# aexoden/snesimage

Measured on AMD Instinct MI355X. Metric: candidate palettes scored/sec, higher is better.
Workload: dtype f32

## Files before the change

### snesimage_amd/csrc/capi.hip

```cpp
#include "../../include/snesimage_hip.h"
#include "kernels.hpp"
#include "kernels_opt.hpp"
#include "kernels_fast.hpp"
#include "kernels_sparse.hpp"
#include "kernels_sparse2.hpp"
#include "kernels_batch.hpp"
#include "kernels_shared.hpp"
#include "kernels_tile.hpp"
#include "kernels_level.hpp"
#include "kernels_char.hpp"
#include "kernels_char_set.hpp"
#include "kernels_guide.hpp"
#include "kernels_guide_lab.hpp"
#include "kernels_guide_window.hpp"
#include "kernels_guide_set_window.hpp"

#include <hip/hip_runtime.h>

#include <atomic>
#include <cmath>
#include <cstdio>
#include <cstdlib>
#include <cstring>
#include <string>
// ... 121 lines not shown
    std::vector<Lane> extra; uint32_t nlanes = 2; hipEvent_t ev_ready = nullptr;
    struct Sparse {
        bool lpt = true;
        bool down1 = true;
        bool counters_cleared = false;
        uint32_t h2q_max = 512;
        bool down_tiles = true;
        uint32_t h0_min = 1024;
        bool base_down_side = false;
        uint32_t h0_grid = 8192;
        hipStream_t h0_stream[8] = {}; hipEvent_t ev_scan[8] = {}, ev_h0[8] = {}, ev_hn[8] = {}, ev_vn[8] = {};
        bool v0_aside = true;
        hipEvent_t ev_v0[8] = {};
        bool vn_aside = true;
        uint32_t tiles_grid = 4096;
        uint32_t down1_grid = 32768;
        bool vsplit = true;
        uint32_t scan4_max = 2048;
        uint32_t hgrid = 8192;
        bool weight_mask = true;
        bool h_planes = true;
        bool debug_poison = false;
        bool dedup = true; uint32_t dedup_min = 1024; int *holder = nullptr; bool holder_dirty = false;
        bool enabled = false, side = true; uint32_t min_n = 1; uint32_t cap = 0, lanes = 0;
        SparseGeom S{};
        float *store = nullptr, *cand_tab = nullptr, *cand_lab = nullptr, *ckf = nullptr, *ckh = nullptr; long long zeros_off = 0; uint32_t *bitmap = nullptr; double *cka = nullptr, *part = nullptr;
        CandMeta *meta = nullptr; unsigned int *items = nullptr; int *item_count = nullptr; long long item_stride = 0; int *order = nullptr, *first = nullptr;
        uint4 *plist = nullptr; int *plist_count = nullptr; bool plist_valid = false;
        hipStream_t base_stream = nullptr; hipEvent_t ev_base_in = nullptr, ev_base_h = nullptr, ev_base_done = nullptr, ev_base_narrow = nullptr;
        uint8_t *dmaps = nullptr, *dmapsC4 = nullptr;
        uint8_t *bmap = nullptr, *bmapC4 = nullptr, *bcand = nullptr; unsigned long long *dpack = nullptr; double *ckd = nullptr; uint32_t slot_ci = 0;
        float *rec_lab = nullptr;
        int base_sp = -1, base_si = -1;
        struct Ahead { uint8_t *bmap = nullptr, *bmapC4 = nullptr, *bcand = nullptr; unsigned long long *dpack = nullptr; double *ckd = nullptr; float *btab = nullptr, *blab = nullptr, *rec_lab = nullptr; int *ok = nullptr;
                       hipEvent_t ev = nullptr; bool on = true, have = false; int sp = -1, si = -1; unsigned long long epoch = 0; } ahead;
    } sp;
    uint8_t *d_cand = nullptr; uint32_t cand_cap = 0;
    uint8_t *d_cand_sel = nullptr;
    double *d_errs = nullptr, *d_errs_sel = nullptr;
    double *d_inc_err = nullptr;
    StepResult *d_last = nullptr;
    double *d_scratch_err = nullptr;
    uint8_t *d_dummy_cand = nullptr;
    KmeansWork km{};
    double *d_tile_cost = nullptr; int *d_tile_any = nullptr; unsigned int *d_tile_moved = nullptr;

// ... 448 lines not shown
            Dn.orig = c->d_orig; Dn.tile_pal = c->d_tile_pal; Dn.pal_rgb8 = c->d_pal_rgb8; Dn.cand_tab = ah.btab; Dn.maps = ah.bmap; Dn.mapsC4 = ah.bmapC4;
            Dn.W = (int)c->W; Dn.H = (int)c->H; Dn.sub_size = (int)c->sub_size; Dn.ncol = c->ncol; Dn.slot_ci = (uint32_t)(np * (int)c->sub_size + ni);
            Dn.rec_pack = ah.dpack; Dn.ck_out = ah.ckd; Dn.excl_sub = np; Dn.excl_si = ni; Dn.excl_j0 = nj0;
            if (c->perceptual) {
                hipLaunchKernelGGL(k_candidate_lab, dim3(1), dim3(64), 0, bs, ah.btab, 1, c->d_lab_eotf, ah.blab);
                Dn.pal_lab = c->d_pal_lab; Dn.cand_lab = ah.blab; Dn.lab_eotf = c->d_lab_eotf; Dn.perceptual = 1; Dn.rec_lab = ah.rec_lab;
                if (c->dither4) hipLaunchKernelGGL((k_dither4_lab<1>), dim3(1), dim3(512), 0, bs, Dn); else hipLaunchKernelGGL((k_dither<true, 0, 1>), dim3(1), dim3(128), 0, bs, Dn);
            } else
            if (c->dither4 && c->sub_size == 15) hipLaunchKernelGGL((k_dither4<15, 1>), dim3(1), dim3(512), 0, bs, Dn);
            else if (c->dither4 && c->sub_size == 16) hipLaunchKernelGGL((k_dither4<16, 1>), dim3(1), dim3(512), 0, bs, Dn);
            else if (c->dither4) hipLaunchKernelGGL((k_dither4<0, 1>), dim3(1), dim3(512), 0, bs, Dn);
            else if (c->sub_size == 15) hipLaunchKernelGGL((k_dither<false, 15, 1>), dim3(1), dim3(128), 0, bs, Dn);
            else if (c->sub_size == 16) hipLaunchKernelGGL((k_dither<false, 16, 1>), dim3(1), dim3(128), 0, bs, Dn);
            else hipLaunchKernelGGL((k_dither<false, 0, 1>), dim3(1), dim3(128), 0, bs, Dn);
            HIPCHK(hipGetLastError());
            HIPCHK(hipEventRecord(ah.ev, bs));
            ah.have = true; ah.sp = np; ah.si = ni; ah.epoch = c->epoch;
        }
        sp.plist_valid = true;
    }
    return SNES_OK;
}

int32_t sparse_score_chunk(snesimage_ctx *c, uint32_t lane, hipStream_t stream, const uint8_t *d_rgb5, uint32_t nc, double *d_errors, int err_stride, int err_offset, int list0 = -1) {
    auto &sp = c->sp;
    const Geom &G = c->G;
    SparseParams P = sparse_params(c, lane);
    P.is_base = 0; P.ncand = (int)nc; P.k0 = (int)(lane * sp.cap);
    if (list0 >= 0) { P.holder = sp.holder; P.list0 = list0; }
    if (sp.debug_poison) HIPCHK(hipMemsetAsync(sp.store + (size_t)P.k0 * sp.S.cand_stride, 0xff, sizeof(float) * (size_t)sp.S.cand_stride * nc, stream));
    snesimage_ctx::TimingRec tr{}; tr.n = nc;
    if (c->timing) { for (int i = 0; i < 6; i++) HIPCHK(hipEventCreate(&tr.ev[i])); if (c->timing == 1) HIPCHK(hipEventRecord(tr.ev[0], stream)); }
    if (list0 >= 0) hipLaunchKernelGGL(k_candidate_tables_mark, dim3((nc + 63) / 64), dim3(64), 0, stream, d_rgb5, (int)nc, c->d_eotf, sp.cand_tab + 8 * (size_t)P.k0, sp.holder, list0);
    else
    hipLaunchKernelGGL(k_candidate_tables, dim3((nc + 63) / 64), dim3(64), 0, stream, d_rgb5, (int)nc, c->d_eotf, sp.cand_tab + 8 * (size_t)P.k0);
    if (c->dither) {
        if (c->perceptual) {
            hipLaunchKernelGGL(k_candidate_lab, dim3((nc + 63) / 64), dim3(64), 0, stream, sp.cand_tab + 8 * (size_t)P.k0, (int)nc, c->d_lab_eotf, sp.cand_lab + 3 * (size_t)P.k0);
            hipLaunchKernelGGL(k_dither_first_lab, dim3(nc), dim3(256), 0, stream, P);
        } else
        hipLaunchKernelGGL(k_dither_first, dim3((nc + 15) / 16), dim3(1024), 0, stream, P);
        DitherParams Dp{};
        Dp.orig = c->d_orig; Dp.tile_pal = c->d_tile_pal; Dp.pal_rgb8 = c->d_pal_rgb8; Dp.cand_tab = sp.cand_tab + 8 * (size_t)P.k0;
        Dp.maps = const_cast<uint8_t *>(P.maps); Dp.mapsC4 = const_cast<uint8_t *>(P.mapsC4);
        Dp.W = (int)c->W; Dp.H = (int)c->H; Dp.sub_size = (int)c->sub_size; Dp.ncol = c->ncol; Dp.slot_ci = sp.slot_ci;
        Dp.first_group = sp.first; Dp.first_k0 = P.k0; Dp.ck_in = sp.ckd; Dp.bmap = sp.bmap; Dp.bmapC4 = sp.bmapC4; Dp.rec_in = c->dither_rec ? sp.dpack : nullptr;
        if (c->sp.lpt) {
            hipLaunchKernelGGL(k_sparse_order, dim3(1), dim3(1024), 0, stream, P, sp.order + P.k0); Dp.order = sp.order + P.k0;
        }
        if (c->perceptual) {
            Dp.pal_lab = c->d_pal_lab; Dp.cand_lab = sp.cand_lab + 3 * (size_t)P.k0; Dp.lab_eotf = c->d_lab_eotf; Dp.perceptual = 1;
            if (c->dither4 && nc <= c->dither4_max) hipLaunchKernelGGL((k_dither4_lab<2>), dim3(nc), dim3(512), 0, stream, Dp); else hipLaunchKernelGGL((k_dither<true, 0, 2>), dim3(nc), dim3(128), 0, stream, Dp);
        } else
        if (c->dither4 && nc <= c->dither4_max && c->sub_size == 15) hipLaunchKernelGGL((k_dither4<15, 2>), dim3(nc), dim3(512), 0, stream, Dp);
        else if (c->dither4 && nc <= c->dither4_max && c->sub_size == 16) hipLaunchKernelGGL((k_dither4<16, 2>), dim3(nc), dim3(512), 0, stream, Dp);
        else if (c->dither4 && nc <= c->dither4_max) hipLaunchKernelGGL((k_dither4<0, 2>), dim3(nc), dim3(512), 0, stream, Dp);
// ... 71 lines not shown
    }
    if (vn_aside) {
        hipStream_t hs = sp.h0_stream[lane];
        HIPCHK(hipStreamWaitEvent(hs, sp.ev_hn[lane], 0));
        HIPCHK(hipStreamWaitEvent(hs, sp.ev_base_narrow, 0));
        hipLaunchKernelGGL(k_sparse_v, dim3((nc * 3 + 7) / 8, (unsigned)(G.nscales - P.s_first)), dim3(256), 0, hs, P);
        HIPCHK(hipEventRecord(sp.ev_vn[lane], hs));
    }
    if (v0_aside) {
        if (sp.side) HIPCHK(hipStreamWaitEvent(stream, sp.ev_base_narrow, 0));
        if (P.s_first < G.nscales) hipLaunchKernelGGL(k_sparse_v, dim3((nc * 3 + 7) / 8, (unsigned)(G.nscales - P.s_first)), dim3(256), 0, stream, P);
        if (P.s_first > 1) hipLaunchKernelGGL(k_sparse_v2_from, dim3(nc * 3, (unsigned)(P.s_first - 1)), dim3(256), 0, stream, P, 1);
    } else {
    if (c->timing) HIPCHK(hipEventRecord(tr.ev[3], stream));
    hipLaunchKernelGGL(k_sparse_v2, dim3(nc * 3, (unsigned)P.s_first), dim3(256), 0, stream, P);
    if (c->timing) HIPCHK(hipEventRecord(tr.ev[4], stream));
    }
    if (vn_aside) HIPCHK(hipStreamWaitEvent(stream, sp.ev_vn[lane], 0));
    else if (!v0_aside) {
    if (sp.side) HIPCHK(hipStreamWaitEvent(stream, sp.ev_base_narrow, 0));
    if (P.s_first < G.nscales) hipLaunchKernelGGL(k_sparse_v, dim3((nc * 3 + 7) / 8, (unsigned)(G.nscales - P.s_first)), dim3(256), 0, stream, P);
    }
    if (v0_aside) HIPCHK(hipStreamWaitEvent(stream, sp.ev_v0[lane], 0));
    hipLaunchKernelGGL(k_final_score_wave, dim3((nc + 3) / 4), dim3(256), 0, stream, sp.part + (size_t)P.k0 * G.nscales * 18, (int)nc, G, d_errors, err_stride, err_offset, P.item_count, (int)kItemLists);
    if (c->dither) {
        uint8_t *bm = lane == 0 ? c->d_bestmap : c->extra[lane - 1].d_bestmap; BestRec *br = lane == 0 ? c->d_bestrec : c->extra[lane - 1].d_bestrec;
        hipLaunchKernelGGL(k_keep_best, dim3(1), dim3(1024), 0, stream, d_errors, err_stride, err_offset, (int)nc, P.maps, (int)c->npx, br, bm);
    }
    HIPCHK(hipGetLastError());
    if (c->timing) { tr.light = c->timing != 1; if (!tr.light) HIPCHK(hipEventRecord(tr.ev[5], stream)); c->t_pending.push_back(tr); }
    return SNES_OK;
}

struct LaneScope {
    snesimage_ctx *c; snesimage_ctx::Lane *L;
    LaneScope(snesimage_ctx *c_, snesimage_ctx::Lane *L_) : c(c_), L(L_) { swap(); }
    ~LaneScope() { swap(); }
    void swap() { std::swap(c->stream, L->stream); std::swap(c->d_work, L->d_work); std::swap(c->d_cand_tab, L->d_cand_tab); std::swap(c->d_cand_lab, L->d_cand_lab);
                  std::swap(c->d_part, L->d_part); std::swap(c->d_maps, L->d_maps); std::swap(c->d_mapsT, L->d_mapsT); std::swap(c->d_mapsC4, L->d_mapsC4); std::swap(c->d_mapsR4, L->d_mapsR4);
                  std::swap(c->d_bestmap, L->d_bestmap); std::swap(c->d_bestrec, L->d_bestrec); }
};

int32_t score_list(snesimage_ctx *c, const uint8_t *d_rgb5, uint32_t n, double *d_errors, int err_stride, int err_offset, int sp, int si, uint8_t *d_maps_out) {
    uint32_t chunk = (c->dither || c->perceptual) ? (n + c->nlanes - 1) / c->nlanes : n;
    if (chunk < 64) chunk = 64;
    if (chunk > c->chunk) chunk = c->chunk;
    if (c->tied_call && chunk > 1024) chunk = 1024;
    const bool sparse = c->sp.enabled && !c->tied_call && !d_maps_out && sp >= 0 && n >= c->sp.min_n && c->pack_mode == (c->dither ? 1 : 2) && !(c->dither && c->sub_size == 1);
    const uint32_t nchunks = (n + chunk - 1) / chunk;
    const uint32_t nl = nchunks < c->nlanes ? nchunks : c->nlanes;
    CHECK(alloc_workspace(c, sparse ? 1 : chunk, nl));
    CHECK(ensure_tables(c));
    CHECK(ensure_source(c));
    if (sparse) {
        CHECK(sparse_alloc(c, chunk, nl));
        if (c->dither && (c->sp.base_sp != sp || c->sp.base_si != si)) c->sp.plist_valid = false;
        CHECK(sparse_base_pass(c, sp, si, n));
        c->sp.base_sp = sp; c->sp.base_si = si;
    }
    if (c->dither) { hipLaunchKernelGGL(k_reset_best, dim3(1), dim3(64), 0, c->stream, c->d_bestrecs_all, (int)c->nlanes); c->best_valid = true; }
    const bool dedup = sparse && !c->dither && c->sp.dedup && n >= c->sp.dedup_min;
    if (dedup) {
        if (!c->sp.holder) { HIPCHK(dmalloc(&c->sp.holder, sizeof(int) * kDedupColours)); c->sp.holder_dirty = true; }
        if (c->sp.holder_dirty) {
            HIPCHK(hipStreamSynchronize(c->stream));
            for (auto &L : c->extra) HIPCHK(hipStreamSynchronize(L.stream));
            HIPCHK(hipMemsetAsync(c->sp.holder, kNoHolder & 0xff, sizeof(int) * kDedupColours, c->stream));
        }
        c->sp.holder_dirty = true;
    }
    if (nl > 1) {
        HIPCHK(hipEventRecord(c->ev_ready, c->stream));
        for (uint32_t l = 1; l < nl; l++) HIPCHK(hipStreamWaitEvent(c->extra[l - 1].stream, c->ev_ready, 0));
    }
    uint32_t i = 0;
    for (uint32_t c0 = 0; c0 < n; c0 += chunk, i++) {
        const uint32_t nc = (n - c0 < chunk) ? (n - c0) : chunk;
        const uint32_t lane = i % nl;
        uint8_t *mo = d_maps_out ? d_maps_out + (size_t)c0 * c->npx : nullptr;
        const int eo = err_offset + (int)c0 * err_stride;
        if (sparse) { CHECK(sparse_score_chunk(c, lane, lane == 0 ? c->stream : c->extra[lane - 1].stream, d_rgb5 + 3 * (size_t)c0, nc, d_errors, err_stride, eo, dedup ? (int)c0 : -1)); continue; }
        if (lane == 0) CHECK(score_chunk(c, d_rgb5 + 3 * (size_t)c0, nc, d_errors, err_stride, eo, sp, si, mo));
        else { LaneScope ls(c, &c->extra[lane - 1]); CHECK(score_chunk(c, d_rgb5 + 3 * (size_t)c0, nc, d_errors, err_stride, eo, sp, si, mo)); }
    }
    for (uint32_t l = 1; l < nl; l++) {
        HIPCHK(hipEventRecord(c->extra[l - 1].done, c->extra[l - 1].stream));
        HIPCHK(hipStreamWaitEvent(c->stream, c->extra[l - 1].done, 0));
    }
    if (dedup) {
        hipLaunchKernelGGL(k_dedup_copy, dim3(1), dim3(1024), 0, c->stream, d_rgb5, (int)n, c->sp.holder, d_errors, err_stride, err_offset);
        HIPCHK(hipGetLastError());
        c->sp.holder_dirty = false;
    }
    return SNES_OK;
}

int32_t ensure_map(snesimage_ctx *c);

int32_t do_optimize(snesimage_ctx *c, bool may_skip = false) {
    CHECK(ensure_tables(c));
    if (!c->dither) {
        c->pack_valid = false;
        CHECK(run_prep(c, 0, -1, -1));
    } else {
        CHECK(alloc_workspace(c, 1));
        if (c->perceptual) CHECK(ensure_source(c));
        hipLaunchKernelGGL(k_candidate_tables, dim3(1), dim3(64), 0, c->stream, c->d_dummy_cand, 1, c->d_eotf, c->d_cand_tab);
        hipLaunchKernelGGL(k_candidate_slot, dim3(1), dim3(64), 0, c->stream, c->d_cand_tab, 1, 0xffffffffu);
        DitherParams Dp{};
        Dp.orig = c->d_orig; Dp.tile_pal = c->d_tile_pal; Dp.pal_rgb8 = c->d_pal_rgb8; Dp.pal_lab = c->d_pal_lab; Dp.cand_tab = c->d_cand_tab; Dp.cand_lab = c->d_cand_lab;
        Dp.lab_eotf = c->d_lab_eotf; Dp.maps = c->d_map; Dp.skip = may_skip ? c->d_skip : nullptr;
        Dp.W = (int)c->W; Dp.H = (int)c->H; Dp.sub_size = (int)c->sub_size; Dp.ncol = c->ncol; Dp.slot_ci = 0xffffffffu; Dp.perceptual = c->perceptual ? 1 : 0;
        launch_dither(c, Dp, 1);
// ... 165 lines not shown
    if (const char *e = getenv("SNES_BASE_STREAM")) c->sp.side = atoi(e) != 0;
    if (const char *e = getenv("SNES_LPT")) c->sp.lpt = atoi(e) != 0;
    if (const char *e = getenv("SNES_DOWN1")) c->sp.down1 = atoi(e) != 0;
    if (const char *e = getenv("SNES_DITHER4")) c->dither4 = atoi(e) != 0;
    if (const char *e = getenv("SNES_DITHERW")) c->ditherw = atoi(e) != 0;
    if (const char *e = getenv("SNES_DITHER_AHEAD")) c->sp.ahead.on = atoi(e) != 0;
    if (const char *e = getenv("SNES_DITHER_REC")) c->dither_rec = atoi(e) != 0;
    if (const char *e = getenv("SNES_DITHER4_MAX")) { int v = atoi(e); if (v >= 0) c->dither4_max = (uint32_t)v; }
    if (const char *e = getenv("SNES_DOWN1_GRID")) { int v = atoi(e); if (v >= 64) c->sp.down1_grid = (uint32_t)v; }
    if (const char *e = getenv("SNES_VSPLIT")) c->sp.vsplit = atoi(e) != 0;
    if (const char *e = getenv("SNES_DOWN_TILES")) c->sp.down_tiles = atoi(e) != 0;
    if (const char *e = getenv("SNES_V0_ASIDE")) c->sp.v0_aside = atoi(e) != 0;
    if (const char *e = getenv("SNES_VN_ASIDE")) c->sp.vn_aside = atoi(e) != 0;
    if (const char *e = getenv("SNES_H0_GRID")) { int v = atoi(e); if (v >= 16) c->sp.h0_grid = (uint32_t)v; }
    if (const char *e = getenv("SNES_H0_MIN")) { int v = atoi(e); if (v >= 0) c->sp.h0_min = (uint32_t)v; }
    if (const char *e = getenv("SNES_TILES_GRID")) { int v = atoi(e); if (v >= 64) c->sp.tiles_grid = (uint32_t)v; }
    if (const char *e = getenv("SNES_SCAN4_MAX")) { int v = atoi(e); if (v >= 0) c->sp.scan4_max = (uint32_t)v; }
    if (const char *e = getenv("SNES_H2Q_MAX")) { int v = atoi(e); if (v >= 0) c->sp.h2q_max = (uint32_t)v; }
    if (const char *e = getenv("SNES_HGRID")) { int v = atoi(e); if (v >= 1) c->sp.hgrid = (uint32_t)v; }
    if (const char *e = getenv("SNES_SPARSE_MIN")) { int v = atoi(e); if (v >= 1) c->sp.min_n = (uint32_t)v; }
    if (const char *e = getenv("SNES_DEDUP")) c->sp.dedup = atoi(e) != 0;
    if (const char *e = getenv("SNES_WEIGHT_MASK")) c->sp.weight_mask = atoi(e) != 0;
    if (const char *e = getenv("SNES_H_PLANES")) c->sp.h_planes = atoi(e) != 0;
    if (const char *e = getenv("SNES_DEBUG_POISON")) c->sp.debug_poison = atoi(e) != 0;
    if (const char *e = getenv("SNES_DEDUP_MIN")) { int v = atoi(e); if (v >= 1) c->sp.dedup_min = (uint32_t)v; }
    Geom &G = c->G;
    G.W = (int)w; G.H = (int)h; G.nscales = 0;
    int P2 = 8;
    while (P2 < (int)h) P2 *= 2;
    for (int s = 0; s < kMaxScales; s++) {
        if (s > 0 && (G.sw[s - 1] < 8 || G.th[s - 1] < 8)) break;
        G.sw[s] = (int)w >> s; G.th[s] = s == 0 ? (int)h : (G.th[s - 1] + 1) / 2; G.sh[s] = s == 0 ? (int)h : P2 >> s; G.nscales = s + 1;
    }
    long long off = 0, soff = 0;
    for (int s = 0; s < G.nscales; s++) {
        long long N = (long long)G.sw[s] * G.sh[s];
        G.src_off[s] = soff; soff += 3 * N;
        if (s >= 1) { G.off_xyb[s] = off; off += 3 * N; G.off_xybT[s] = off; off += 3 * N; } else { G.off_xyb[s] = 0; G.off_xybT[s] = 0; }
        G.off_hout[s] = off; off += 9 * N;
    }
    G.cand_stride = off;
    for (int s = 0; s < G.nscales; s++) if ((G.sw[s] % 64) == 0 && (G.th[s] % 64) == 0 && G.th[s] == G.sh[s]) c->fast_mask |= 1 << s;
    if (const char *e = getenv("SNES_NO_FAST")) { if (atoi(e)) c->fast_mask = 0; }
    c->src_floats = (size_t)soff;

    int32_t rc = SNES_OK;
// ... 547 lines not shown
```

### snesimage_amd/csrc/kernels.hpp

```cpp
#pragma once
#include "color.hpp"

namespace snes {

constexpr int kMaxScales = SSIM2_NUM_SCALES;
constexpr int kBlurRadius = 5;

SNES_HD long long idx_c4(int x, int y, int H) { return ((long long)(x >> 2) * H + y) * 4 + (x & 3); }
SNES_HD long long idx_r4(int x, int y, int W) { return ((long long)(y >> 2) * W + x) * 4 + (y & 3); }
SNES_HD long long idx_xt4(int x, int y, int H) { return ((((long long)(x >> 6) * (H >> 2)) + (y >> 2)) << 8) + ((x & 63) << 2) + (y & 3); }

struct BlurK {
    float n2[3];
    float d1[3];
};

struct Geom {
    int W, H, nscales;
    int sw[kMaxScales], sh[kMaxScales];
    int th[kMaxScales];
    long long off_xyb[kMaxScales], off_xybT[kMaxScales], off_hout[kMaxScales];
    long long cand_stride;
    long long src_off[kMaxScales];
};
// ... 56 lines not shown
    uint32_t rgb8 = 0;
    if (i < ncol) rgb8 = rgb5_to_rgb8(colors[3 * i], colors[3 * i + 1], colors[3 * i + 2]);
    float r = eotf[rgb8 & 0xff], g = eotf[(rgb8 >> 8) & 0xff], b = eotf[(rgb8 >> 16) & 0xff];
    float X, Y, B;
    linear_to_positive_xyb(r, g, b, X, Y, B);
    pal_rgb8[i] = rgb8;
    pal_lin[3 * i] = r; pal_lin[3 * i + 1] = g; pal_lin[3 * i + 2] = b;
    pal_xyb[3 * i] = X; pal_xyb[3 * i + 1] = Y; pal_xyb[3 * i + 2] = B;
}

__device__ __forceinline__ void candidate_tables_body(const uint8_t *__restrict__ rgb5, int n, const float *__restrict__ eotf, float *__restrict__ cand_tab) {
    int k = blockIdx.x * blockDim.x + threadIdx.x;
    if (k >= n) return;
    uint32_t rgb8 = rgb5_to_rgb8(rgb5[3 * k], rgb5[3 * k + 1], rgb5[3 * k + 2]);
    float r = eotf[rgb8 & 0xff], g = eotf[(rgb8 >> 8) & 0xff], b = eotf[(rgb8 >> 16) & 0xff];
    float X, Y, B;
    linear_to_positive_xyb(r, g, b, X, Y, B);
    float *o = cand_tab + 8 * (size_t)k;
    o[0] = r; o[1] = g; o[2] = b; o[3] = X; o[4] = Y; o[5] = B; o[6] = __uint_as_float(rgb8); o[7] = 0.0f;
}

constexpr int kDedupColours = 32768;
constexpr int kNoHolder = 0x7f7f7f7f;
__device__ __forceinline__ int dedup_key(uint32_t rgb8) {
    const uint32_t r = (rgb8 >> 3) & 31u, g = (rgb8 >> 11) & 31u, b = (rgb8 >> 19) & 31u;
    return rgb5_to_rgb8(r, g, b) == (rgb8 & 0x00ffffffu) ? (int)(r | (g << 5) | (b << 10)) : -1;
}
__device__ __forceinline__ void candidate_tables_mark_body(const uint8_t *__restrict__ rgb5, int n, const float *__restrict__ eotf, float *__restrict__ cand_tab, int *__restrict__ holder, int list0) {
    candidate_tables_body(rgb5, n, eotf, cand_tab);
    const int k = blockIdx.x * blockDim.x + threadIdx.x;
    if (k >= n) return;
    const int key = dedup_key(rgb5_to_rgb8(rgb5[3 * k], rgb5[3 * k + 1], rgb5[3 * k + 2]));
    if (key >= 0) atomicMin(&holder[key], list0 + k);
}
__device__ __forceinline__ bool dedup_is_duplicate(const int *__restrict__ holder, uint32_t rgb8, int idx) {
    const int key = dedup_key(rgb8);
    return key >= 0 && holder[key] != idx;
}
__device__ __forceinline__ void dedup_copy_body(const uint8_t *__restrict__ rgb5, int n, int *__restrict__ holder, double *__restrict__ errors, int err_stride, int err_offset) {
    for (int j = threadIdx.x; j < n; j += blockDim.x) {
        const int key = dedup_key(rgb5_to_rgb8(rgb5[3 * j], rgb5[3 * j + 1], rgb5[3 * j + 2]));
        if (key < 0) continue;
        const int h = holder[key];
        if (h != j && (unsigned)h < (unsigned)n) errors[(size_t)err_offset + (size_t)j * err_stride] = errors[(size_t)err_offset + (size_t)h * err_stride];
    }
    __syncthreads();
    for (int j = threadIdx.x; j < n; j += blockDim.x) {
        const int key = dedup_key(rgb5_to_rgb8(rgb5[3 * j], rgb5[3 * j + 1], rgb5[3 * j + 2]));
        if (key >= 0) holder[key] = kNoHolder;
    }
}

constexpr uint32_t kTiedSlot = 0x7d000000u;
__device__ __forceinline__ bool slot_hit(uint32_t ci, uint32_t slot_ci, uint32_t ncol) {
    if ((slot_ci >> 24) != (kTiedSlot >> 24)) return ci == slot_ci;
    return ci < ncol && ci % ((slot_ci >> 8) & 0xffu) == (slot_ci & 0xffu);
}

struct PrepParams {
    const uint8_t *orig; const uint8_t *tile_pal; const uint32_t *pal_rgb8; uint8_t *map;
    unsigned long long *pack, *packT, *packC4, *packR4;
    uint8_t *subC4, *subR4;
    const float *labpx; const float *pal_lab;
    int W, H, sub_size, ncol, mode, sp, si, perceptual;
    int *zero; int nzero;
};
// ... 584 lines not shown
    for (int ch = 0; ch < 3; ch++)
        for (int s = 0; s < G.nscales; s++) {
            const double *p = part + (((size_t)c * G.nscales + s) * 3 + ch) * 6;
            const double opp = 1.0 / (double)((size_t)G.sw[s] * G.th[s]);
            double avg_ssim[2] = {opp * p[0], sqrt(sqrt(opp * p[1]))};
            double avg_edge[4] = {opp * p[2], sqrt(sqrt(opp * p[3])), opp * p[4], sqrt(sqrt(opp * p[5]))};
            for (int n = 0; n < 2; n++) {
                ssim = fma(kSsim2Weight[i], fabs(avg_ssim[n]), ssim); i++;
                ssim = fma(kSsim2Weight[i], fabs(avg_edge[n]), ssim); i++;
                ssim = fma(kSsim2Weight[i], fabs(avg_edge[n + 2]), ssim); i++;
            }
        }
    ssim *= SSIM2_SCORE_SCALE;
    ssim = fma(SSIM2_SCORE_C3 * ssim * ssim, ssim, fma(SSIM2_SCORE_C1, ssim, SSIM2_SCORE_C2 * ssim * ssim));
    if (ssim > 0.0) ssim = fma(pow(ssim, SSIM2_SCORE_EXP), SSIM2_SCORE_GAIN, SSIM2_SCORE_MAX);
    else ssim = SSIM2_SCORE_MAX;
    errors[(size_t)err_offset + (size_t)c * err_stride] = 100.0 - ssim;
}

__device__ __forceinline__ double readlane_f64(double v, int l) {
    const int lo = __builtin_amdgcn_readlane(__double2loint(v), l), hi = __builtin_amdgcn_readlane(__double2hiint(v), l);
    return __hiloint2double(hi, lo);
}
__device__ __forceinline__ void final_score_wave_body(const double *__restrict__ part, int ncand, const Geom &G, double *__restrict__ errors, int err_stride, int err_offset, int *__restrict__ zero, int nzero) {
    const int gt = blockIdx.x * blockDim.x + threadIdx.x;
    if (zero && gt < nzero) zero[gt] = 0;
    const int lane = threadIdx.x & 63, c = __builtin_amdgcn_readfirstlane(gt >> 6);
    if (c >= ncand) return;
    const int ns = G.nscales, npair = 3 * ns;
    double term[6] = {0.0, 0.0, 0.0, 0.0, 0.0, 0.0};
    if (lane < npair) {
        const int ch = lane / ns, s = lane - ch * ns;
        const double *p = part + (((size_t)c * ns + s) * 3 + ch) * 6;
        const double opp = 1.0 / (double)((size_t)G.sw[s] * G.th[s]);
        term[0] = opp * p[0]; term[1] = opp * p[2]; term[2] = opp * p[4];
        term[3] = sqrt(sqrt(opp * p[1])); term[4] = sqrt(sqrt(opp * p[3])); term[5] = sqrt(sqrt(opp * p[5]));
    }
    double ssim = 0.0;
    int i = 0;
    for (int l = 0; l < npair; l++) {
#pragma unroll
        for (int t = 0; t < 6; t++) { ssim = fma(kSsim2Weight[i], fabs(readlane_f64(term[t], l)), ssim); i++; }
    }
    if (lane != 0) return;
    ssim *= SSIM2_SCORE_SCALE;
    ssim = fma(SSIM2_SCORE_C3 * ssim * ssim, ssim, fma(SSIM2_SCORE_C1, ssim, SSIM2_SCORE_C2 * ssim * ssim));
    if (ssim > 0.0) ssim = fma(pow(ssim, SSIM2_SCORE_EXP), SSIM2_SCORE_GAIN, SSIM2_SCORE_MAX);
    else ssim = SSIM2_SCORE_MAX;
    errors[(size_t)err_offset + (size_t)c * err_stride] = 100.0 - ssim;
}

__global__ void k_candidate_tables(const uint8_t *__restrict__ rgb5, int n, const float *__restrict__ eotf, float *__restrict__ cand_tab) { candidate_tables_body(rgb5, n, eotf, cand_tab); }
__global__ void k_candidate_tables_mark(const uint8_t *__restrict__ rgb5, int n, const float *__restrict__ eotf, float *__restrict__ cand_tab, int *__restrict__ holder, int list0) { candidate_tables_mark_body(rgb5, n, eotf, cand_tab, holder, list0); }
__global__ __launch_bounds__(1024) void k_dedup_copy(const uint8_t *__restrict__ rgb5, int n, int *__restrict__ holder, double *__restrict__ errors, int err_stride, int err_offset) { dedup_copy_body(rgb5, n, holder, errors, err_stride, err_offset); }
__global__ __launch_bounds__(256) void k_prep(PrepParams P) { prep_body(P); }
__global__ void k_final_score(const double *__restrict__ part, int ncand, Geom G, double *__restrict__ errors, int err_stride, int err_offset, int *__restrict__ zero = nullptr, int nzero = 0) {
    final_score_body(part, ncand, G, errors, err_stride, err_offset, zero, nzero);
}
__global__ __launch_bounds__(256) void k_final_score_wave(const double *__restrict__ part, int ncand, Geom G, double *__restrict__ errors, int err_stride, int err_offset, int *__restrict__ zero = nullptr, int nzero = 0) {
    final_score_wave_body(part, ncand, G, errors, err_stride, err_offset, zero, nzero);
}

}
```

### snesimage_amd/csrc/window_host.inc

```

struct WindowPolicy {
    double calls = 0.0, accepts = 0.0;
    uint32_t next(uint32_t used, uint32_t acc, uint32_t lo, uint32_t hi, uint32_t ranks, uint32_t taken, double weight = 1.0) {
        calls = 0.85 * calls + used; accepts = 0.85 * accepts + acc;
        const double p = (accepts + 0.5) / (calls + 8.0);
        double best = -1.0; uint32_t best_k = lo;
        for (uint32_t k = lo; k <= hi; k = k < 4 ? 2 * k : k + (k < 32 * ranks ? 4 : 8) * ranks) {
            const double through = (1.0 - std::pow(1.0 - p, (double)k)) / p, rate = through / (15.0 + weight * (double)k / ranks);
            if (rate > best) { best = rate; best_k = k; }
        }
        if (!acc && used == taken) { const uint32_t twice = 2 * taken > hi ? hi : 2 * taken; if (twice > best_k) best_k = twice; }
        return best_k;
    }
};

struct WindowRec {
    unsigned char *h_blob = nullptr, *d_blob = nullptr;
    snes::BatchArgs *h_args = nullptr, *d_args = nullptr;
    snes::WindowSlot *h_slots = nullptr, *d_slots = nullptr;
    snes::WindowResult *h_res = nullptr, *d_res = nullptr;
    snes::StepResult *h_log = nullptr, *d_log = nullptr;
    uint8_t *d_cand = nullptr; double *d_errs = nullptr;
    hipEvent_t ev[7] = {nullptr, nullptr, nullptr, nullptr, nullptr, nullptr, nullptr}, args = nullptr, done = nullptr;
    uint32_t K = 0, stride = 0; bool logged = false;
// ... 36 lines not shown
struct WindowGen {
    uint32_t n;
    void (*next)(const snesimage_ctx *c, uint32_t *palette, uint32_t *index);
    int32_t (*generate)(snesimage_ctx *c, WindowRec &r, uint32_t K, uint32_t n, double *d_errors);
};

void window_release_child(snesimage_ctx *k) {
    k->d_orig = nullptr; k->d_tile_pal = nullptr; k->d_colors = nullptr; k->d_map = nullptr; k->d_eotf = nullptr; k->d_lab_eotf = nullptr;
    k->d_pal_rgb8 = nullptr; k->d_pal_lin = nullptr; k->d_pal_xyb = nullptr; k->d_pal_lab = nullptr; k->d_lin0 = nullptr; k->d_img1 = nullptr; k->d_img1T = nullptr; k->d_mu1 = nullptr; k->d_sd1 = nullptr;
    k->d_a1 = nullptr; k->d_a1R4 = nullptr; k->d_r1 = nullptr; k->d_r1R4 = nullptr; k->d_img1C4 = nullptr; k->d_mu1R4 = nullptr; k->d_sd1R4 = nullptr; k->d_labpx = nullptr; k->d_labpxT = nullptr; k->d_target = nullptr; k->d_labpx_t = nullptr; k->d_labpxT_t = nullptr;
    k->d_inc_err = nullptr; k->d_last = nullptr; k->d_scratch_err = nullptr; k->d_dummy_cand = nullptr;
    if (k->pack_borrowed) { k->d_pack = nullptr; k->d_packC4 = nullptr; k->d_packR4 = nullptr; k->d_subC4 = nullptr; k->d_subR4 = nullptr; }
    k->stream = nullptr; k->own_stream = nullptr;
    snesimage_destroy(k);
}

int32_t window_make_child(snesimage_ctx *c, snesimage_ctx **out) {
    std::unique_ptr<snesimage_ctx, void (*)(snesimage_ctx *)> k(new snesimage_ctx(), window_release_child);
    k->device = c->device; k->W = c->W; k->H = c->H; k->sub_count = c->sub_count; k->sub_size = c->sub_size; k->user_size = c->sub_size; k->flags = c->flags;  k->ncol = c->ncol;
    k->dither_rec = c->dither_rec; k->dither4 = c->dither4; k->dither4_max = c->dither4_max; k->ditherw = c->ditherw; k->sp.ahead.on = false;
    k->dither = c->dither; k->perceptual = c->perceptual; k->nes = c->nes; k->G = c->G; k->K = c->K; k->npx = c->npx; k->src_floats = c->src_floats; k->fast_mask = c->fast_mask;
    k->chunk = kMemberCand; k->nlanes = 1;
    k->sp.enabled = true; k->sp.side = false; k->sp.lpt = c->sp.lpt; k->sp.down1 = c->sp.down1; k->sp.h2q_max = c->sp.h2q_max; k->sp.scan4_max = c->sp.scan4_max; k->sp.vsplit = c->sp.vsplit; k->sp.down_tiles = c->sp.down_tiles; k->sp.tiles_grid = c->sp.tiles_grid; k->sp.h0_min = c->sp.h0_min; k->sp.hgrid = c->sp.hgrid; k->sp.min_n = 1;
    k->sp.weight_mask = c->sp.weight_mask; k->sp.h_planes = c->sp.h_planes; k->sp.debug_poison = c->sp.debug_poison;
    k->d_orig = c->d_orig; k->d_tile_pal = c->d_tile_pal; k->d_colors = c->d_colors; k->d_map = c->d_map; k->d_eotf = c->d_eotf; k->d_lab_eotf = c->d_lab_eotf;
    k->d_pal_rgb8 = c->d_pal_rgb8; k->d_pal_lin = c->d_pal_lin; k->d_pal_xyb = c->d_pal_xyb; k->d_pal_lab = c->d_pal_lab;
    k->d_img1C4 = c->d_img1C4; k->d_mu1R4 = c->d_mu1R4; k->d_sd1R4 = c->d_sd1R4; k->d_a1R4 = c->d_a1R4; k->d_r1R4 = c->d_r1R4; k->d_labpx = c->d_labpx; k->d_labpxT = c->d_labpxT; k->d_target = c->d_target; k->d_labpx_t = c->d_labpx_t; k->d_labpxT_t = c->d_labpxT_t; k->od_n = c->od_n; memcpy(k->od_tab, c->od_tab, sizeof k->od_tab);
    k->d_inc_err = c->d_inc_err; k->d_last = c->d_last;
    k->stream = c->stream;
    k->tables_valid = true; k->src_valid = true;
    if (c->dither) {
        k->pack_borrowed = true;
        k->d_pack = c->d_pack; k->d_packC4 = c->d_packC4; k->d_packR4 = c->d_packR4; k->d_subC4 = c->d_subC4; k->d_subR4 = c->d_subR4;
    } else {
        HIPCHK(dmalloc(&k->d_pack, c->npx * 8));
        HIPCHK(dmalloc(&k->d_packC4, c->npx * 8));
        HIPCHK(dmalloc(&k->d_packR4, c->npx * 8));
    }
    CHECK(sparse_alloc(k.get(), kMemberCand));
    *out = k.release();
    return SNES_OK;
}

size_t window_slots_bytes(uint32_t K) { return (sizeof(snes::WindowSlot) * (size_t)K + 15) & ~(size_t)15; }
size_t window_blob_bytes(uint32_t cap) { return window_slots_bytes(cap) + sizeof(snes::BatchArgs) * (size_t)cap; }
void window_rec_free(WindowRec &r) {
    if (r.h_blob) (void)hipHostFree(r.h_blob); if (r.h_res) (void)hipHostFree(r.h_res); if (r.h_log) (void)hipHostFree(r.h_log);
// ... 281 lines not shown
```

Baseline: 3.245 million.

## Fuse dedup copy into final scoring and tag holder entries to skip resets

Duplicate candidates are now resolved inside the final score kernel when the whole batch is one chunk: each candidate reads the partial sums of its holder, so the single-block dedup copy kernel no longer runs. Holder entries carry a per-call tag in the high byte, so the holder table is memset and stream-synchronised only once every ~126 calls instead of every call. This removes a serial 1-block launch, a 128 KB memset and host stream syncs per call. In exchange it adds a holder lookup in the score kernel and depends on tag arithmetic staying correct across calls.

```diff
diff --git a/profiles/front_of_call.py b/profiles/front_of_call.py
--- /dev/null
+++ b/profiles/front_of_call.py
@@ -0,0 +1,78 @@
+#!/usr/bin/env python3
+import argparse
+import glob
+import json
+import os
+import subprocess
+import sys
+import tempfile
+
+ap = argparse.ArgumentParser()
+ap.add_argument("out")
+ap.add_argument("--rounds", type=int, default=3)
+ap.add_argument("--leg", action="append", required=True)
+ap.add_argument("--outputs", action="store_true")
+ap.add_argument("--side", action="store_true")
+ap.add_argument("--channel", action="store_true")
+ap.add_argument("--limit", type=int, default=240, help="seconds per run")
+args = ap.parse_args()
+
+legs = []
+for spec in args.leg:
+    name, rest = spec.split("=", 1)
+    parts = rest.split(",")
+    legs.append((name, os.path.abspath(parts[0]), dict(p.split("=", 1) for p in parts[1:])))
+res = {"what": "python bench.py [args], the legs alternating on one MI355X in one session, one process per run", "legs": {n: {"tree": os.path.relpath(t), "env": e} for n, t, e in legs},
+       "runs": [], "outputs": {}, "side_figures_ms_per_step": {}}
+
+
+def save():
+    json.dump(res, open(args.out, "w"), indent=1)
+
+
+def bench(tree, env, extra):
+    cmd = ["timeout", "-k", "10", str(args.limit), sys.executable, "bench.py"] + extra
+    p = subprocess.run(cmd, cwd=tree, env=dict(os.environ, **env), stdout=subprocess.PIPE, stderr=subprocess.PIPE, text=True)
+    if p.returncode != 0:
+        print(p.stdout[-2000:], p.stderr[-4000:], file=sys.stderr)
+        res["failed"] = {"cmd": cmd, "tree": tree, "rc": p.returncode}
+        save()
+        sys.exit("run failed with status %d: nothing more is started" % p.returncode)
+    line = [ln for ln in p.stdout.splitlines() if ln.startswith("{")][-1]
+    return json.loads(line)
+
+
+for rnd in range(1, args.rounds + 1):
+    for label, extra in (("default", []), ("s20", ["--gpus", "1", "--steps", "20", "--warmup", "5"])):
+        for name, tree, env in legs:
+            d = bench(tree, env, extra)
+            r = {"leg": name, "round": rnd, "invocation": label, "args": extra, "env": env, "ms_per_step": d["ms_per_step"], "value": d.get("value"), "unit": d.get("unit"),
+                 "steps": d.get("steps"), "warmup": d.get("warmup"), "library": d.get("library") or d.get("config", {}).get("library")}
+            res["runs"].append(r)
+            print("round %d %-8s %-12s %.4f ms" % (rnd, label, name, d["ms_per_step"]), flush=True)
+            save()
+
+if args.outputs or args.side or args.channel:
+    two = legs[:2]
+    (na, ta, ea), (nb, tb, eb) = two
+    for cfg in ("rgb", "perceptual", "dither", "images"):
+        cargs = [] if cfg == "rgb" else ["--config", cfg]
+        if args.outputs and cfg != "images":
+            with tempfile.TemporaryDirectory() as tmp:
+                ms = {}
+                for n, t, e in two:
+                    ms[n] = bench(t, e, cargs + ["--steps", "20", "--warmup", "5", "--dump-outputs", os.path.join(tmp, n)])["ms_per_step"]
+                fa = sorted(os.path.basename(f) for f in glob.glob(os.path.join(tmp, na, "*.npy")))
+                fb = sorted(os.path.basename(f) for f in glob.glob(os.path.join(tmp, nb, "*.npy")))
+                same = {f: open(os.path.join(tmp, na, f), "rb").read() == open(os.path.join(tmp, nb, f), "rb").read() for f in fa}
+                res["outputs"][cfg] = {"arrays": fa, "same_names": fa == fb, "identical": same, "all_identical": bool(fa) and fa == fb and all(same.values()), "ms_per_step_20": ms}
+                print("outputs %-10s %s" % (cfg, res["outputs"][cfg]), flush=True)
+                save()
+        if args.side and cfg != "rgb":
+            res["side_figures_ms_per_step"][cfg] = {n: bench(t, e, cargs + ["--steps", "40", "--warmup", "5"])["ms_per_step"] for n, t, e in two}
+            print("side %-10s %s" % (cfg, res["side_figures_ms_per_step"][cfg]), flush=True)
+            save()
+    if args.channel:
+        res["channel_calls_ms_per_call"] = {n: bench(t, e, ["--full", "--steps", "40", "--warmup", "5"])["channel_calls"]["ms_per_call"] for n, t, e in two}
+        print("side channel_calls %s" % res["channel_calls_ms_per_call"], flush=True)
+        save()
diff --git a/snesimage_amd/csrc/capi.hip b/snesimage_amd/csrc/capi.hip
--- a/snesimage_amd/csrc/capi.hip
+++ b/snesimage_amd/csrc/capi.hip
@@ -167,6 +167,7 @@
         bool h_planes = true;
         bool debug_poison = false;
         bool dedup = true; uint32_t dedup_min = 1024; int *holder = nullptr; bool holder_dirty = false;
+        bool dedup_fuse = true; int dedup_tag = kDedupTags;
         bool enabled = false, side = true; uint32_t min_n = 1; uint32_t cap = 0, lanes = 0;
         SparseGeom S{};
         float *store = nullptr, *cand_tab = nullptr, *cand_lab = nullptr, *ckf = nullptr, *ckh = nullptr; long long zeros_off = 0; uint32_t *bitmap = nullptr; double *cka = nullptr, *part = nullptr;
@@ -661,16 +662,16 @@
     return SNES_OK;
 }
 
-int32_t sparse_score_chunk(snesimage_ctx *c, uint32_t lane, hipStream_t stream, const uint8_t *d_rgb5, uint32_t nc, double *d_errors, int err_stride, int err_offset, int list0 = -1) {
+int32_t sparse_score_chunk(snesimage_ctx *c, uint32_t lane, hipStream_t stream, const uint8_t *d_rgb5, uint32_t nc, double *d_errors, int err_stride, int err_offset, int list0 = -1, int tag = 0, bool whole_list = false) {
     auto &sp = c->sp;
     const Geom &G = c->G;
     SparseParams P = sparse_params(c, lane);
     P.is_base = 0; P.ncand = (int)nc; P.k0 = (int)(lane * sp.cap);
-    if (list0 >= 0) { P.holder = sp.holder; P.list0 = list0; }
+    if (list0 >= 0) { P.holder = sp.holder; P.list0 = tag + list0; }
     if (sp.debug_poison) HIPCHK(hipMemsetAsync(sp.store + (size_t)P.k0 * sp.S.cand_stride, 0xff, sizeof(float) * (size_t)sp.S.cand_stride * nc, stream));
     snesimage_ctx::TimingRec tr{}; tr.n = nc;
     if (c->timing) { for (int i = 0; i < 6; i++) HIPCHK(hipEventCreate(&tr.ev[i])); if (c->timing == 1) HIPCHK(hipEventRecord(tr.ev[0], stream)); }
-    if (list0 >= 0) hipLaunchKernelGGL(k_candidate_tables_mark, dim3((nc + 63) / 64), dim3(64), 0, stream, d_rgb5, (int)nc, c->d_eotf, sp.cand_tab + 8 * (size_t)P.k0, sp.holder, list0);
+    if (list0 >= 0) hipLaunchKernelGGL(k_candidate_tables_mark, dim3((nc + 63) / 64), dim3(64), 0, stream, d_rgb5, (int)nc, c->d_eotf, sp.cand_tab + 8 * (size_t)P.k0, sp.holder, tag + list0);
     else
     hipLaunchKernelGGL(k_candidate_tables, dim3((nc + 63) / 64), dim3(64), 0, stream, d_rgb5, (int)nc, c->d_eotf, sp.cand_tab + 8 * (size_t)P.k0);
     if (c->dither) {
@@ -788,6 +789,9 @@
     if (P.s_first < G.nscales) hipLaunchKernelGGL(k_sparse_v, dim3((nc * 3 + 7) / 8, (unsigned)(G.nscales - P.s_first)), dim3(256), 0, stream, P);
     }
     if (v0_aside) HIPCHK(hipStreamWaitEvent(stream, sp.ev_v0[lane], 0));
+    if (whole_list) hipLaunchKernelGGL(k_final_score_wave_dedup, dim3((nc + 3) / 4), dim3(256), 0, stream, sp.part + (size_t)P.k0 * G.nscales * 18, (int)nc, G, d_errors, err_stride, err_offset, P.item_count, (int)kItemLists,
+                                       sp.holder, sp.cand_tab + 8 * (size_t)P.k0, tag);
+    else
     hipLaunchKernelGGL(k_final_score_wave, dim3((nc + 3) / 4), dim3(256), 0, stream, sp.part + (size_t)P.k0 * G.nscales * 18, (int)nc, G, d_errors, err_stride, err_offset, P.item_count, (int)kItemLists);
     if (c->dither) {
         uint8_t *bm = lane == 0 ? c->d_bestmap : c->extra[lane - 1].d_bestmap; BestRec *br = lane == 0 ? c->d_bestrec : c->extra[lane - 1].d_bestrec;
@@ -826,15 +830,23 @@
     }
     if (c->dither) { hipLaunchKernelGGL(k_reset_best, dim3(1), dim3(64), 0, c->stream, c->d_bestrecs_all, (int)c->nlanes); c->best_valid = true; }
     const bool dedup = sparse && !c->dither && c->sp.dedup && n >= c->sp.dedup_min;
+    int dedup_tag = 0;
     if (dedup) {
         if (!c->sp.holder) { HIPCHK(dmalloc(&c->sp.holder, sizeof(int) * kDedupColours)); c->sp.holder_dirty = true; }
-        if (c->sp.holder_dirty) {
-            HIPCHK(hipStreamSynchronize(c->stream));
-            for (auto &L : c->extra) HIPCHK(hipStreamSynchronize(L.stream));
+        const bool tagged = c->sp.dedup_fuse && n < (1u << 24);
+        const bool start_over = tagged ? c->sp.dedup_tag <= 1 : c->sp.dedup_tag != kDedupTags;
+        if (c->sp.holder_dirty || start_over) {
+            if (c->sp.holder_dirty) {
+                HIPCHK(hipStreamSynchronize(c->stream));
+                for (auto &L : c->extra) HIPCHK(hipStreamSynchronize(L.stream));
+            }
             HIPCHK(hipMemsetAsync(c->sp.holder, kNoHolder & 0xff, sizeof(int) * kDedupColours, c->stream));
+            c->sp.dedup_tag = kDedupTags;
         }
         c->sp.holder_dirty = true;
-    }
+        if (tagged) dedup_tag = --c->sp.dedup_tag << 24;
+    }
+    const bool dedup_fused = dedup && dedup_tag != 0 && nchunks == 1;
     if (nl > 1) {
         HIPCHK(hipEventRecord(c->ev_ready, c->stream));
         for (uint32_t l = 1; l < nl; l++) HIPCHK(hipStreamWaitEvent(c->extra[l - 1].stream, c->ev_ready, 0));
@@ -845,7 +857,7 @@
         const uint32_t lane = i % nl;
         uint8_t *mo = d_maps_out ? d_maps_out + (size_t)c0 * c->npx : nullptr;
         const int eo = err_offset + (int)c0 * err_stride;
-        if (sparse) { CHECK(sparse_score_chunk(c, lane, lane == 0 ? c->stream : c->extra[lane - 1].stream, d_rgb5 + 3 * (size_t)c0, nc, d_errors, err_stride, eo, dedup ? (int)c0 : -1)); continue; }
+        if (sparse) { CHECK(sparse_score_chunk(c, lane, lane == 0 ? c->stream : c->extra[lane - 1].stream, d_rgb5 + 3 * (size_t)c0, nc, d_errors, err_stride, eo, dedup ? (int)c0 : -1, dedup_tag, dedup_fused)); continue; }
         if (lane == 0) CHECK(score_chunk(c, d_rgb5 + 3 * (size_t)c0, nc, d_errors, err_stride, eo, sp, si, mo));
         else { LaneScope ls(c, &c->extra[lane - 1]); CHECK(score_chunk(c, d_rgb5 + 3 * (size_t)c0, nc, d_errors, err_stride, eo, sp, si, mo)); }
     }
@@ -853,8 +865,10 @@
         HIPCHK(hipEventRecord(c->extra[l - 1].done, c->extra[l - 1].stream));
         HIPCHK(hipStreamWaitEvent(c->stream, c->extra[l - 1].done, 0));
     }
+    if (dedup_fused) c->sp.holder_dirty = false;
+    else
     if (dedup) {
-        hipLaunchKernelGGL(k_dedup_copy, dim3(1), dim3(1024), 0, c->stream, d_rgb5, (int)n, c->sp.holder, d_errors, err_stride, err_offset);
+        hipLaunchKernelGGL(k_dedup_copy, dim3(1), dim3(1024), 0, c->stream, d_rgb5, (int)n, c->sp.holder, d_errors, err_stride, err_offset, dedup_tag);
         HIPCHK(hipGetLastError());
         c->sp.holder_dirty = false;
     }
@@ -1066,6 +1080,7 @@
     if (const char *e = getenv("SNES_DEDUP")) c->sp.dedup = atoi(e) != 0;
     if (const char *e = getenv("SNES_WEIGHT_MASK")) c->sp.weight_mask = atoi(e) != 0;
     if (const char *e = getenv("SNES_H_PLANES")) c->sp.h_planes = atoi(e) != 0;
+    if (const char *e = getenv("SNES_DEDUP_FUSE")) c->sp.dedup_fuse = atoi(e) != 0;
     if (const char *e = getenv("SNES_DEBUG_POISON")) c->sp.debug_poison = atoi(e) != 0;
     if (const char *e = getenv("SNES_DEDUP_MIN")) { int v = atoi(e); if (v >= 1) c->sp.dedup_min = (uint32_t)v; }
     Geom &G = c->G;
diff --git a/snesimage_amd/csrc/kernels.hpp b/snesimage_amd/csrc/kernels.hpp
--- a/snesimage_amd/csrc/kernels.hpp
+++ b/snesimage_amd/csrc/kernels.hpp
@@ -102,6 +102,7 @@
 
 constexpr int kDedupColours = 32768;
 constexpr int kNoHolder = 0x7f7f7f7f;
+constexpr int kDedupTags = 0x7f;
 __device__ __forceinline__ int dedup_key(uint32_t rgb8) {
     const uint32_t r = (rgb8 >> 3) & 31u, g = (rgb8 >> 11) & 31u, b = (rgb8 >> 19) & 31u;
     return rgb5_to_rgb8(r, g, b) == (rgb8 & 0x00ffffffu) ? (int)(r | (g << 5) | (b << 10)) : -1;
@@ -117,11 +118,11 @@
     const int key = dedup_key(rgb8);
     return key >= 0 && holder[key] != idx;
 }
-__device__ __forceinline__ void dedup_copy_body(const uint8_t *__restrict__ rgb5, int n, int *__restrict__ holder, double *__restrict__ errors, int err_stride, int err_offset) {
+__device__ __forceinline__ void dedup_copy_body(const uint8_t *__restrict__ rgb5, int n, int *__restrict__ holder, double *__restrict__ errors, int err_stride, int err_offset, int tag = 0) {
     for (int j = threadIdx.x; j < n; j += blockDim.x) {
         const int key = dedup_key(rgb5_to_rgb8(rgb5[3 * j], rgb5[3 * j + 1], rgb5[3 * j + 2]));
         if (key < 0) continue;
-        const int h = holder[key];
+        const int h = holder[key] - tag;
         if (h != j && (unsigned)h < (unsigned)n) errors[(size_t)err_offset + (size_t)j * err_stride] = errors[(size_t)err_offset + (size_t)h * err_stride];
     }
     __syncthreads();
@@ -752,16 +753,23 @@
     const int lo = __builtin_amdgcn_readlane(__double2loint(v), l), hi = __builtin_amdgcn_readlane(__double2hiint(v), l);
     return __hiloint2double(hi, lo);
 }
-__device__ __forceinline__ void final_score_wave_body(const double *__restrict__ part, int ncand, const Geom &G, double *__restrict__ errors, int err_stride, int err_offset, int *__restrict__ zero, int nzero) {
+__device__ __forceinline__ void final_score_wave_body(const double *__restrict__ part, int ncand, const Geom &G, double *__restrict__ errors, int err_stride, int err_offset, int *__restrict__ zero, int nzero,
+                                                      const int *__restrict__ holder = nullptr, const float *__restrict__ cand_tab = nullptr, int tag = 0) {
     const int gt = blockIdx.x * blockDim.x + threadIdx.x;
     if (zero && gt < nzero) zero[gt] = 0;
     const int lane = threadIdx.x & 63, c = __builtin_amdgcn_readfirstlane(gt >> 6);
     if (c >= ncand) return;
+    int src = c;
+    if (holder) {
+        const int key = dedup_key(__float_as_uint(cand_tab[8 * (size_t)c + 6]));
+        if (key >= 0) { const int h = holder[key] - tag; if ((unsigned)h < (unsigned)ncand) src = h; }
+        src = __builtin_amdgcn_readfirstlane(src);
+    }
     const int ns = G.nscales, npair = 3 * ns;
     double term[6] = {0.0, 0.0, 0.0, 0.0, 0.0, 0.0};
     if (lane < npair) {
         const int ch = lane / ns, s = lane - ch * ns;
-        const double *p = part + (((size_t)c * ns + s) * 3 + ch) * 6;
+        const double *p = part + (((size_t)src * ns + s) * 3 + ch) * 6;
         const double opp = 1.0 / (double)((size_t)G.sw[s] * G.th[s]);
         term[0] = opp * p[0]; term[1] = opp * p[2]; term[2] = opp * p[4];
         term[3] = sqrt(sqrt(opp * p[1])); term[4] = sqrt(sqrt(opp * p[3])); term[5] = sqrt(sqrt(opp * p[5]));
@@ -782,7 +790,7 @@
 
 __global__ void k_candidate_tables(const uint8_t *__restrict__ rgb5, int n, const float *__restrict__ eotf, float *__restrict__ cand_tab) { candidate_tables_body(rgb5, n, eotf, cand_tab); }
 __global__ void k_candidate_tables_mark(const uint8_t *__restrict__ rgb5, int n, const float *__restrict__ eotf, float *__restrict__ cand_tab, int *__restrict__ holder, int list0) { candidate_tables_mark_body(rgb5, n, eotf, cand_tab, holder, list0); }
-__global__ __launch_bounds__(1024) void k_dedup_copy(const uint8_t *__restrict__ rgb5, int n, int *__restrict__ holder, double *__restrict__ errors, int err_stride, int err_offset) { dedup_copy_body(rgb5, n, holder, errors, err_stride, err_offset); }
+__global__ __launch_bounds__(1024) void k_dedup_copy(const uint8_t *__restrict__ rgb5, int n, int *__restrict__ holder, double *__restrict__ errors, int err_stride, int err_offset, int tag = 0) { dedup_copy_body(rgb5, n, holder, errors, err_stride, err_offset, tag); }
 __global__ __launch_bounds__(256) void k_prep(PrepParams P) { prep_body(P); }
 __global__ void k_final_score(const double *__restrict__ part, int ncand, Geom G, double *__restrict__ errors, int err_stride, int err_offset, int *__restrict__ zero = nullptr, int nzero = 0) {
     final_score_body(part, ncand, G, errors, err_stride, err_offset, zero, nzero);
@@ -790,5 +798,9 @@
 __global__ __launch_bounds__(256) void k_final_score_wave(const double *__restrict__ part, int ncand, Geom G, double *__restrict__ errors, int err_stride, int err_offset, int *__restrict__ zero = nullptr, int nzero = 0) {
     final_score_wave_body(part, ncand, G, errors, err_stride, err_offset, zero, nzero);
 }
-
-}
+__global__ __launch_bounds__(256) void k_final_score_wave_dedup(const double *__restrict__ part, int ncand, Geom G, double *__restrict__ errors, int err_stride, int err_offset, int *__restrict__ zero, int nzero,
+                                                                const int *__restrict__ holder, const float *__restrict__ cand_tab, int tag) {
+    final_score_wave_body(part, ncand, G, errors, err_stride, err_offset, zero, nzero, holder, cand_tab, tag);
+}
+
+}
diff --git a/snesimage_amd/csrc/window_host.inc b/snesimage_amd/csrc/window_host.inc
--- a/snesimage_amd/csrc/window_host.inc
+++ b/snesimage_amd/csrc/window_host.inc
@@ -82,7 +82,7 @@
     k->dither = c->dither; k->perceptual = c->perceptual; k->nes = c->nes; k->G = c->G; k->K = c->K; k->npx = c->npx; k->src_floats = c->src_floats; k->fast_mask = c->fast_mask;
     k->chunk = kMemberCand; k->nlanes = 1;
     k->sp.enabled = true; k->sp.side = false; k->sp.lpt = c->sp.lpt; k->sp.down1 = c->sp.down1; k->sp.h2q_max = c->sp.h2q_max; k->sp.scan4_max = c->sp.scan4_max; k->sp.vsplit = c->sp.vsplit; k->sp.down_tiles = c->sp.down_tiles; k->sp.tiles_grid = c->sp.tiles_grid; k->sp.h0_min = c->sp.h0_min; k->sp.hgrid = c->sp.hgrid; k->sp.min_n = 1;
-    k->sp.weight_mask = c->sp.weight_mask; k->sp.h_planes = c->sp.h_planes; k->sp.debug_poison = c->sp.debug_poison;
+    k->sp.weight_mask = c->sp.weight_mask; k->sp.h_planes = c->sp.h_planes; k->sp.dedup_fuse = c->sp.dedup_fuse; k->sp.debug_poison = c->sp.debug_poison;
     k->d_orig = c->d_orig; k->d_tile_pal = c->d_tile_pal; k->d_colors = c->d_colors; k->d_map = c->d_map; k->d_eotf = c->d_eotf; k->d_lab_eotf = c->d_lab_eotf;
     k->d_pal_rgb8 = c->d_pal_rgb8; k->d_pal_lin = c->d_pal_lin; k->d_pal_xyb = c->d_pal_xyb; k->d_pal_lab = c->d_pal_lab;
     k->d_img1C4 = c->d_img1C4; k->d_mu1R4 = c->d_mu1R4; k->d_sd1R4 = c->d_sd1R4; k->d_a1R4 = c->d_a1R4; k->d_r1R4 = c->d_r1R4; k->d_labpx = c->d_labpx; k->d_labpxT = c->d_labpxT; k->d_target = c->d_target; k->d_labpx_t = c->d_labpx_t; k->d_labpxT_t = c->d_labpxT_t; k->od_n = c->od_n; memcpy(k->od_tab, c->od_tab, sizeof k->od_tab);
```

Result: faster. 3.287 million (median of 6 runs) (+1.3%).
